# MCG-NJU/LinK

Measured on AMD Instinct MI355X. Metric: voxels/s through one LinK (3x7)^3 block, 100k active voxels C=64, higher is better.
Workload: dtype f32

## Files before the change

### link_amd/csrc/dense_batch_impl.h

```cpp
#include <stdlib.h>

#include <type_traits>
#include <vector>

#include "dense_batch_common.h"
#include "dense_gather.h"
#include "dense_io.h"

namespace DC_IO_NS {
using namespace link;

#include "dense_k1_impl.h"
#include "dense_k2_cfg.h"
#include "dense_gather_quad_impl.h"

static_assert(DC_ST_AUX == 16, "the S rows must leave the L2 (sc1) for the in-launch hand-off K1 -> K2");

struct dc_bt_frame_t {
  const void *feats; const int4 *coords; int4 *slots; uint32_t *cnt; int32_t *cell_n; int32_t *vcell; float *S; int32_t *hdr;
  void *out; int64_t n;
};
struct dc_bt_frames_t { dc_bt_frame_t f[DC_BT_MAX]; };
struct dc_bt_par_t {
  const float *w_pre, *pre_ln_w, *pre_ln_b, *w_pos, *ln_w, *ln_b;
// ... 143 lines not shown
struct dc_bt_k2_args_t {
  dc_bt_frames_t fr;
  dc_bt_par_t p;
  link_dc_grid_t g;
  int nframes, txn, tyn, zsplit, nwg, k1_target;
  int32_t *sync;
};

template <int OP, int R>
__global__ void __launch_bounds__(256 + 64 * (DC_K2Q_CW + (DC_K2Q_PMAP ? 1 : 0)), 4) k_dc_batch_k2(dc_bt_k2_args_t args_by_value) {
  (void)args_by_value;
#if defined(__HIP_DEVICE_COMPILE__)
  static_assert(DC_K2Q_PMAP == 1, "the mapper wave draws the items");
  typedef const __attribute__((address_space(4))) dc_bt_k2_args_t *args_ptr_t;
  constexpr unsigned CTL_THREAD = 256 + 64 * DC_K2Q_CW;
  __shared__ int s_ctl[2];
  const int x = (int)(__builtin_amdgcn_s_getreg((4 - 1) << 11 | 0 << 6 | 20) & 7u);
  int t_next = 0;
  if (threadIdx.x == CTL_THREAD) {
    args_ptr_t a = (args_ptr_t)__builtin_amdgcn_kernarg_segment_ptr();
    int32_t *sy = a->sync;
    const int per = (a->nwg + 7) >> 3;
    if (DC_BT_PROF)
      bt_row(a->p.dbg2, (unsigned long long)a->nframes * (8 * per) + blockIdx.x, 9999, 0, __builtin_amdgcn_s_memrealtime(), 0, 0, blockIdx.x);
    const int t = __hip_atomic_fetch_add(&sy[bt_cursor(x)], 1, __ATOMIC_RELAXED, __HIP_MEMORY_SCOPE_AGENT);
    t_next = __hip_atomic_fetch_add(&sy[bt_cursor(x)], 1, __ATOMIC_RELAXED, __HIP_MEMORY_SCOPE_AGENT);
    int f = t < a->nframes * per ? t / per : -1;
    if (f >= 0 && !bt_wait_ge(sy, bt_k1(f), a->k1_target)) f = -1;
    s_ctl[0] = f; s_ctl[1] = f >= 0 ? (t - f * per) * 8 + x : 0;
  }
  __syncthreads();
  for (;;) {
    args_ptr_t a = (args_ptr_t)__builtin_amdgcn_kernarg_segment_ptr();
    asm volatile("" : "+s"(a));
    const int f = __builtin_amdgcn_readfirstlane(s_ctl[0]), bid = __builtin_amdgcn_readfirstlane(s_ctl[1]);
    if (f < 0) break;
    const unsigned long long tq0 = DC_BT_PROF ? __builtin_amdgcn_s_memrealtime() : 0;
    __syncthreads();
    {
      const link_dc_grid_t g = a->g;
      unsigned tidx = threadIdx.x;
      asm volatile("" : "+v"(tidx));
      dc_k2q_body<OP, R, false, true>(a->fr.f[f].S, a->fr.f[f].cell_n, a->fr.f[f].slots, a->p.w_pos, nullptr, a->p.ln_w, a->p.ln_b, a->p.cg,
                                      1.0f, a->p.eps, a->fr.f[f].n, g, a->txn, a->tyn, a->zsplit, a->nwg, a->fr.f[f].out, nullptr, bid, tidx);
    }
    if (threadIdx.x == CTL_THREAD) {
      const unsigned long long tq1 = DC_BT_PROF ? __builtin_amdgcn_s_memrealtime() : 0;
      int32_t *sy = a->sync;
      const int per = (a->nwg + 7) >> 3;
      const int t = t_next;
      int fn = t < a->nframes * per ? t / per : -1;
      if (fn >= 0) {
        t_next = __hip_atomic_fetch_add(&sy[bt_cursor(x)], 1, __ATOMIC_RELAXED, __HIP_MEMORY_SCOPE_AGENT);
        if (!bt_wait_ge(sy, bt_k1(fn), a->k1_target)) fn = -1;
      }
      s_ctl[0] = fn; s_ctl[1] = fn >= 0 ? (t - fn * per) * 8 + x : 0;
      if (DC_BT_PROF) bt_row(a->p.dbg2, (unsigned long long)f * (8 * per) + bid, (unsigned long long)f, (unsigned long long)bid, tq0, tq1, __builtin_amdgcn_s_memrealtime(), (unsigned long long)blockIdx.x);
    }
    __syncthreads();
  }
#endif
}


template <int OP, int R>
static int batch_launch(const dc_bt_host_t &c, const dc_bt_frames_t &fr, const dc_bt_par_t &p, const link_dc_grid_t &g, const link_elk_desc_t &d,
                        int nframes, int64_t nmax) {
  using K1 = dc_k1_cfg<64, OP>;
  using KQ = dc_k2q_cfg<OP, R>;
  using KG = typename dc_k2_cfg<OP, R>::G;
  constexpr int LDS_GRAN = 1280, LDS_GRANS = 128, K1_STATIC = 256, K2_STATIC = 16;
  constexpr int k1_lds = 65 * LDS_GRAN - K1_STATIC;
  constexpr int k2_lds = KQ::LDS_BYTES;
  static_assert(k1_lds >= K1::LDS_BYTES && (k2_lds + K2_STATIC + LDS_GRAN - 1) / LDS_GRAN <= LDS_GRANS - 65, "LDS shaping of the two persistent roles");
  int32_t *sync = c.sync;
  const int64_t vi = (int64_t)g.dim[0] * g.dim[1] * g.dim[2] * g.dim[3];
  const int k1_wgs = c.cus;
  static const int rpw = [] { const char *e = getenv("LINK_DC_BATCH_RPW"); const int v = e ? atoi(e) : 1; return v < 1 ? 1 : (v > 16 ? 16 : v); }();
  int cpw = (int)((vi + (int64_t)k1_wgs * K1::NW * rpw - 1) / ((int64_t)k1_wgs * K1::NW * rpw));
  if (cpw < 1) cpw = 1;
  const int k1_target = (int)((vi + cpw - 1) / cpw);
  const int txn = (g.dim[0] + KG::TX - 1) / KG::TX, tyn = (g.dim[1] + KG::TY - 1) / KG::TY;
  static const int zs_env = [] { const char *e = getenv("LINK_DC_BATCH_ZSPLIT"); const int v = e ? atoi(e) : 1; return v < 1 ? 1 : (v > 8 ? 8 : v); }();
  int zsplit = zs_env;
  if (zsplit > g.dim[2]) zsplit = g.dim[2];
  const int64_t nwg = (int64_t)txn * tyn * g.dim[3] * zsplit;
  if (nwg > (1 << 20)) return LINK_ERR_ARG;
  int wpf = (int)((nmax + 255) / 256);
  if (wpf < 1) wpf = 1;
  (void)hipFuncSetAttribute(reinterpret_cast<const void *>(&k_dc_batch_k1<OP, 2>), hipFuncAttributeMaxDynamicSharedMemorySize, k1_lds);
  (void)hipFuncSetAttribute(reinterpret_cast<const void *>(&k_dc_batch_k2<OP, R>), hipFuncAttributeMaxDynamicSharedMemorySize, k2_lds);
  const int ins_wgs = c.cus;
  const dc_bt_ins_args_t a0{fr, g, nframes, wpf, sync};
  hipLaunchKernelGGL(k_dc_batch_insert, dim3((unsigned)ins_wgs * DC_BT_INS_WAVES), dim3(64), 0, c.sc, a0);
  int rc = check_launch("link_elk_core_dense_forward_batch (insert)");
  if (rc != LINK_OK) return rc;
  hipLaunchKernelGGL((k_dc_batch_k1<OP, 2>), dim3((unsigned)k1_wgs), dim3(64 * K1::NW), k1_lds, c.sa, fr, p, g, nframes, cpw, k1_target, wpf, sync);
  rc = check_launch("link_elk_core_dense_forward_batch (K1)");
  if (rc != LINK_OK) return rc;
  const dc_bt_k2_args_t a2{fr, p, g, nframes, txn, tyn, zsplit, (int)nwg, k1_target, sync};
  static_assert(sizeof(dc_bt_k2_args_t) <= 4096, "kernel arguments");
  hipLaunchKernelGGL((k_dc_batch_k2<OP, R>), dim3((unsigned)c.cus), dim3(KQ::THREADS), k2_lds, c.sb, a2);
  return check_launch("link_elk_core_dense_forward_batch (K2)");
}

int batch_set_launch(const dc_bt_host_t &c, const link_dc_buffers_t *frames, const int64_t *n, int nb, const link_dc_grid_t &g,
                     const link_elk_desc_t &d) {
  const link_dc_buffers_t &b0 = frames[0];
  const dc_bt_par_t p{b0.w_pre, b0.pre_ln_w, b0.pre_ln_b, b0.w_pos, b0.ln_w, b0.ln_b, d.cg, d.eps, c.dbg1, c.dbg2};
  dc_bt_frames_t fr{};
  int64_t nmax = 0;
  for (int i = 0; i < nb; i++) {
    const link_dc_buffers_t &b = frames[i];
    fr.f[i] = dc_bt_frame_t{b.feats, reinterpret_cast<const int4 *>(b.coords), reinterpret_cast<int4 *>(b.slots), b.cnt, b.cell_n, b.vcell, b.S,
                            b.hdr, b.out, n[i]};
    nmax = n[i] > nmax ? n[i] : nmax;
  }
  if (d.op == LINK_OP_COS) return d.r == 3 ? batch_launch<LINK_OP_COS, 3>(c, fr, p, g, d, nb, nmax) : batch_launch<LINK_OP_COS, 2>(c, fr, p, g, d, nb, nmax);
  return d.r == 3 ? batch_launch<LINK_OP_SIN, 3>(c, fr, p, g, d, nb, nmax) : batch_launch<LINK_OP_SIN, 2>(c, fr, p, g, d, nb, nmax);
}
}
```

### link_amd/csrc/dense_fused_impl.h

```cpp
#pragma once
#include <type_traits>

#include "dense_gather.h"
#include "dense_io.h"

namespace DC_IO_NS {
using namespace link;

#include "dense_k1_impl.h"

template <int C, int OP, int NB, bool PIPE>
static int launch_k1p(const link_dc_buffers_t *b, const link_dc_grid_t &g, const link_elk_desc_t &d, int64_t n,
                     bool warm, hipStream_t st) {
  using K = dc_k1_cfg<C, OP>;
  const int64_t vi = (int64_t)g.dim[0] * g.dim[1] * g.dim[2] * g.dim[3];
  int64_t waves = (int64_t)(b->tune.k1_wgs > 0 ? b->tune.k1_wgs : 512) * 4;
  int cpw = (int)((vi + waves - 1) / waves);
  if (cpw < 1) cpw = 1;
  const int64_t wgs = (vi + (int64_t)cpw * K::NW - 1) / ((int64_t)cpw * K::NW);
  int k1_pad = b->tune.k1_lds_pad;
  k1_pad = k1_pad < 0 ? 0 : (k1_pad > 16384 ? 16384 : k1_pad);
  const int lds_k1 = K::LDS_BYTES + k1_pad <= 160 * 1024 ? K::LDS_BYTES + k1_pad : K::LDS_BYTES;
  if (lds_k1 > 64 * 1024)
    (void)hipFuncSetAttribute(reinterpret_cast<const void *>(&k_dc_premix_modsum<C, OP, NB, PIPE>),
// ... 825 lines not shown
    (void)hipFuncSetAttribute(reinterpret_cast<const void *>(&k_dc_gather_demod_own<OP, R, PP, DD>),                  \
                              hipFuncAttributeMaxDynamicSharedMemorySize, KO::LDS_BYTES + k2_pad);                   \
    hipLaunchKernelGGL((k_dc_gather_demod_own<OP, R, PP, DD>), dim3((unsigned)grid), dim3(320), KO::LDS_BYTES + k2_pad, st, b->S, \
                       b->cell_n, reinterpret_cast<const int4 *>(b->slots), b->fin, b->w_pos, b->alpha, b->ln_w,      \
                       b->ln_b, d.cg, d.coord_div, d.eps, n, g, txn, tyn, zsplit, (int)nwg, b->out,                   \
                       reinterpret_cast<unsigned long long *>(b->tune.k2_dbg));                                       \
  } while (0)
    if (pair) { if (div) LINK_K2O(true, true); else LINK_K2O(true, false); }
    else { if (div) LINK_K2O(false, true); else LINK_K2O(false, false); }
#undef LINK_K2O
    return check_launch("link_dc_gather_demod");
  }
  if constexpr (dc_k2q_cfg<OP, R>::FITS) {
    if (pair && !b->alpha && !(b->tune.k2_form & 9) && !k2_single) {
      using KQ = dc_k2q_cfg<OP, R>;
#define LINK_K2Q(DD)                                                                                                  \
  do {                                                                                                                \
    (void)hipFuncSetAttribute(reinterpret_cast<const void *>(&k_dc_gather_demod_quad<OP, R, DD>),                     \
                              hipFuncAttributeMaxDynamicSharedMemorySize, KQ::LDS_BYTES + k2_pad);                   \
    hipLaunchKernelGGL((k_dc_gather_demod_quad<OP, R, DD>), dim3((unsigned)grid), dim3(KQ::THREADS), KQ::LDS_BYTES + k2_pad, st, b->S, \
                       b->cell_n, reinterpret_cast<const int4 *>(b->slots), b->w_pos, b->alpha, b->ln_w, b->ln_b, d.cg, \
                       d.coord_div, d.eps, n, g, txn, tyn, zsplit, (int)nwg, b->out,                                   \
                       reinterpret_cast<unsigned long long *>(b->tune.k2_dbg));                                       \
  } while (0)
      if (div) LINK_K2Q(true); else LINK_K2Q(false);
#undef LINK_K2Q
      return check_launch("link_dc_gather_demod");
    }
  }
  if (!(b->tune.k2_form & 1) && K2::SPLIT_FITS) {
    if (pair) { if (div) LINK_K2S(true, true); else LINK_K2S(true, false); }
    else { if (div) LINK_K2S(false, true); else LINK_K2S(false, false); }
    return check_launch("link_dc_gather_demod");
  }
#undef LINK_K2S
#define LINK_K2(PP, DD)                                                                                               \
  do {                                                                                                                \
// ... 55 lines not shown
```

### link_amd/csrc/dense_gather.h

```cpp
#pragma once
#include "dense_common.h"

namespace link {

template <int C, int P, int R>
struct dc_gather_cfg {
  static constexpr int LPR = C / 4;
  static constexpr int NG = 256 / LPR;
  static constexpr int TY = NG >= 64 ? 8 : (NG >= 16 ? 4 : 2);
  static constexpr int TX = NG / TY;
  static constexpr int HLO = (R == 3) ? 1 : 0;
  static constexpr int HX = TX + R - 1, HY = TY + R - 1;
  static constexpr int NCOL = HX * HY;
  static constexpr int RP = P * C / 4;
  static constexpr int NPC = NCOL * RP;
  static constexpr int PASSES = (NPC + 255) / 256;
  static constexpr int EPW = 64;
  static constexpr int NI = PASSES + 1;
  static constexpr int PLANE_BYTES = PASSES * 256 * 16;
  static constexpr int CNT_BYTES = 4 * 256;
  static constexpr int BUF_BYTES = PLANE_BYTES + CNT_BYTES;
  static constexpr int LDS_BYTES = 3 * BUF_BYTES;
  static_assert(NCOL <= 256, "count image: 4 waves x 64 entries");
  static_assert(NCOL * P * C * 4 + 3 * C * 4 < 65536, "ds_read immediate offsets are 16 bit");
};
// ... 57 lines not shown
        "ds_read_b32 %6, %9 offset:%c16\n\tds_read_b32 %7, %9 offset:%c17\n\t"
        "s_waitcnt lgkmcnt(0)"
        : "=&v"(v0), "=&v"(v1), "=&v"(v2), "=&v"(v3), "=&v"(v4), "=&v"(v5), "=&v"(n0), "=&v"(n1)
        : "v"(ra), "v"(ca), O_(0, 0), O_(0, 1), O_(0, 2), O_(1, 0), O_(1, 1), O_(1, 2), Q_(0), Q_(1)
        : "memory");
    const v4f_t a = v0 + v3, b = v1 + v4, d = v2 + v5;
    cur[0].x += a.x; cur[0].y += a.y; cur[0].z += a.z; cur[0].w += a.w;
    cur[1].x += b.x; cur[1].y += b.y; cur[1].z += b.z; cur[1].w += b.w;
    cur[P - 1].x += d.x; cur[P - 1].y += d.y; cur[P - 1].z += d.z; cur[P - 1].w += d.w;
  }
  cc += (float)n0 + (float)n1 + (float)n2;
#undef O_
#undef Q_
}

template <int C>
__device__ __forceinline__ void dc_read_plane_p2r3(uint32_t ra, uint32_t ca, float4 (&cur)[2], float &cc) {
  using K = dc_gather_cfg<C, 2, 3>;
  constexpr int RB = 2 * C * 4;
#define O_(dx, dy, pp) "i"((((dx) * K::HY + (dy)) * RB) + (pp) * C * 4)
#define Q_(dx, dy) "i"(((dx) * K::HY + (dy)) * 4)
  v4f_t a0, a1, a2, a3, a4, a5, b0, b1, b2, b3, b4, b5;
  int m0, m1, m2, n0, n1, n2;
  asm volatile(
      "ds_read_b128 %0, %18 offset:%c20\n\tds_read_b128 %1, %18 offset:%c21\n\t"
      "ds_read_b128 %2, %18 offset:%c22\n\tds_read_b128 %3, %18 offset:%c23\n\t"
      "ds_read_b128 %4, %18 offset:%c24\n\tds_read_b128 %5, %18 offset:%c25\n\t"
      "ds_read_b32 %6, %19 offset:%c26\n\tds_read_b32 %7, %19 offset:%c27\n\tds_read_b32 %8, %19 offset:%c28\n\t"
      "ds_read_b128 %9, %18 offset:%c29\n\tds_read_b128 %10, %18 offset:%c30\n\t"
      "ds_read_b128 %11, %18 offset:%c31\n\tds_read_b128 %12, %18 offset:%c32\n\t"
      "ds_read_b128 %13, %18 offset:%c33\n\tds_read_b128 %14, %18 offset:%c34\n\t"
      "ds_read_b32 %15, %19 offset:%c35\n\tds_read_b32 %16, %19 offset:%c36\n\tds_read_b32 %17, %19 offset:%c37\n\t"
      "s_waitcnt lgkmcnt(9)"
// ... 44 lines not shown
```

### link_amd/csrc/dense_gather_quad_impl.h

```cpp
#pragma once
#ifndef DC_K2_MAP
#define DC_K2_MAP 1
#endif

#ifndef DC_K2Q_CW
#define DC_K2Q_CW 3
#endif
#ifndef DC_K2Q_PMAP
#define DC_K2Q_PMAP 1
#endif
#ifndef DC_K2Q_EARLY
#define DC_K2Q_EARLY 1
#endif
#ifndef DC_K2Q_RIM
#define DC_K2Q_RIM 1
#endif
#ifndef DC_K2Q_FMA
#define DC_K2Q_FMA 1
#endif

template <int OP, int R>
struct dc_k2q_cfg {
  using K2 = dc_k2_cfg<OP, R>;
  static constexpr int PAR_OFF = K2::SPLIT_LDS_BYTES;
  static constexpr int MAP_OFF = PAR_OFF + 2 * 64 * 4;
  static constexpr int MAP_BYTES = 64 * 4 + 16;
  static constexpr int LDS_BYTES = MAP_OFF + (DC_K2Q_PMAP ? 3 * MAP_BYTES : 0);
  static constexpr int THREADS = 256 + 64 * (DC_K2Q_CW + (DC_K2Q_PMAP ? 1 : 0));
  static constexpr bool FITS = K2::P == 2 && 2 * LDS_BYTES <= 160 * 1024;
};

__device__ __forceinline__ void lds_rd9_b128(uint32_t ar, uint32_t a0, uint32_t a1, v4f_t &r, v4f_t (&x)[2][4]) {
  asm volatile("ds_read_b128 %0, %9\n\t"
               "ds_read_b128 %1, %10\n\tds_read_b128 %2, %10 offset:64\n\tds_read_b128 %3, %10 offset:128\n\tds_read_b128 %4, %10 offset:192\n\t"
               "ds_read_b128 %5, %11\n\tds_read_b128 %6, %11 offset:64\n\tds_read_b128 %7, %11 offset:128\n\tds_read_b128 %8, %11 offset:192\n\t"
               "s_waitcnt lgkmcnt(0)"
               : "=&v"(r), "=&v"(x[0][0]), "=&v"(x[0][1]), "=&v"(x[0][2]), "=&v"(x[0][3]), "=&v"(x[1][0]), "=&v"(x[1][1]),
                 "=&v"(x[1][2]), "=&v"(x[1][3])
// ... 48 lines not shown
    asm volatile("ds_read_b32 %0, %4\n\tds_read_b32 %1, %5\n\tds_read_b32 %2, %6\n\tds_read_b32 %3, %7\n\ts_waitcnt lgkmcnt(0)"
                 : "=&v"(cn[0]), "=&v"(cn[1]), "=&v"(cn[2]), "=&v"(cn[3])
                 : "v"(base + off[0]), "v"(base + off[1]), "v"(base + off[2]), "v"(base + off[3])
                 : "memory");
  } else {
#pragma unroll
    for (int i = 0; i < N; i++) cn[i] = lds_rd_b32(base + off[i]);
  }
}
__device__ __forceinline__ float dc_quad_sum(float v) {
  v += __builtin_bit_cast(float, __builtin_amdgcn_update_dpp(0, __builtin_bit_cast(int, v), 0xB1, 0xF, 0xF, true));
  v += __builtin_bit_cast(float, __builtin_amdgcn_update_dpp(0, __builtin_bit_cast(int, v), 0x4E, 0xF, 0xF, true));
  return v;
}

template <int OP, int R, bool DIV, bool COH = false>
__device__ __forceinline__ void dc_k2q_body(
    const float *__restrict__ S_, const int32_t *__restrict__ cell_n, const int4 *__restrict__ slots,
    const float *__restrict__ w_pos, const float *__restrict__ alpha, const float *__restrict__ ln_w,
    const float *__restrict__ ln_b, int cg, float coord_div, float eps, int64_t n, const link_dc_grid_t &g, int txn, int tyn,
    int zsplit, int nwg, void *__restrict__ out, unsigned long long *__restrict__ dbg, const int bid, const unsigned tidx) {
  using K2 = dc_k2_cfg<OP, R>;
  using KQ = dc_k2q_cfg<OP, R>;
  DC_PROF_PTR(dbg);
  unsigned long long tq0 = dbg ? DC_NOW() : 0, tq_dma = 0, tq_bar = 0, tq_work = 0;
  int tq_rounds = 0;
  using K = typename K2::G;
  constexpr int C = 64, P = 2, TY = K::TY, TX = K::TX, HY = K::HY, HLO = K::HLO;
  constexpr int RB = P * C * 4;
  static_assert(K2::P == 2, "two-part rows");
  extern __shared__ __attribute__((aligned(16))) char lds[];
  const bool producer = tidx < 256;
  const int tid = tidx & 255, lane = tid & 63, wave = __builtin_amdgcn_readfirstlane((tidx & 255) >> 6);
  const int per = (nwg + 7) >> 3;
  const int L = (bid & 7) * per + (bid >> 3);
  if (L >= nwg) return;
  int t = L;
  const int zseg = t % zsplit; t /= zsplit;
#if DC_K2_MAP
  const int per_b = txn * tyn;
  const int b = t / per_b;
  int tt2 = t - b * per_b;
  const int H = (tyn + 1) >> 1;
  int tx, ty;
  if (tt2 < txn * H) { tx = tt2 / H; ty = tt2 - tx * H; }
  else { tt2 -= txn * H; const int H2 = tyn - H; tx = tt2 / H2; ty = H + tt2 - tx * H2; }
#else
  const int ty = t % tyn; t /= tyn;
  const int tx = t % txn;
  const int b = t / txn;
#endif
  const int Dx = g.dim[0], Dy = g.dim[1], Dz = g.dim[2];
  const int PDx = g.pdim[0], PDy = g.pdim[1], PDz = g.pdim[2];
  const int x0 = tx * TX, y0 = ty * TY;
  const int zs = (int)(((long long)Dz * zseg) / zsplit), ze = (int)(((long long)Dz * (zseg + 1)) / zsplit);
  if (zs >= ze) return;
  const int nplanes = (ze - zs) + R - 1;
  const int pz0 = zs + 1 - HLO;
  const uint32_t lds_base = (uint32_t)(size_t)(__attribute__((address_space(3))) char *)lds;
  const uint32_t abuf0 = lds_base + K2::SPLIT_ABUF_OFF, ncnt0 = lds_base + K2::SPLIT_NCNT_OFF;
  if (tidx < 128) {
    float *par = reinterpret_cast<float *>(lds + KQ::PAR_OFF);
    par[tidx] = tidx < 64 ? ln_w[tidx] : ln_b[tidx - 64];
  }
  if (producer) {
    auto col_cell0 = [&](int hx, int hy) {
      int px = x0 + 1 - HLO + hx, py = y0 + 1 - HLO + hy;
      px = px < PDx - 1 ? px : PDx - 1;
      py = py < PDy - 1 ? py : PDy - 1;
// ... 18 lines not shown
    auto cnt_slot = [&](int plane, int pm3) -> uint32_t {
      (void)plane;
      return (uint32_t)(pm3 * K2::SPLIT_BUF_BYTES + K2::SPLIT_PLANE);
    };
    auto issue_cnt = [&](int plane, int pm3) {
      int pz = pz0 + plane;
      pz = pz < PDz - 1 ? pz : PDz - 1;
      const int32_t *csrc = cell_n + cnt_cell0 + pz;
      __builtin_amdgcn_global_load_lds((const __attribute__((address_space(1))) void *)csrc,
                                       (__attribute__((address_space(3))) void *)(lds + cnt_slot(plane, pm3) + wave * 256), 4, 0, COH ? 16 : 0);
    };
    uint32_t rec_cell0;
    int rec_k;
    {
      const int piece = wave * 16 + (lane & 15);
      const int col = piece >> 2;
      rec_k = piece & 3;
      rec_cell0 = col_cell0(col / TY + HLO, col % TY + HLO);
    }
    const char *Sb = reinterpret_cast<const char *>(S_);
    auto issue = [&](int plane, int pm3, bool) {
      int pz = pz0 + plane;
      pz = pz < PDz - 1 ? pz : PDz - 1;
      char *buf = lds + pm3 * K2::SPLIT_BUF_BYTES;
#pragma unroll
      for (int i = 0; i < K::PASSES; i++) {
        const bool surplus = (i * 256 + wave * 64) >= K::NPC;
        const int ii = surplus ? 0 : i;
        const char *src = Sb + (size_t)(surplus ? src_off[0] : src_off[i]) + (size_t)pz * RB;
        __builtin_amdgcn_global_load_lds((const __attribute__((address_space(1))) void *)src,
                                         (__attribute__((address_space(3))) void *)(buf + (ii * 256 + wave * 64) * 16), 16, 0, COH ? 16 : 0);
      }
      issue_cnt(plane, pm3);
      int po = pz0 + plane - (R - 1) + HLO;
      po = po < 0 ? 0 : (po < PDz - 1 ? po : PDz - 1);
      const int4 *rsrc = slots + ((size_t)(rec_cell0 + po) * DC_INL + rec_k);
      if (lane < 16)
        __builtin_amdgcn_global_load_lds((const __attribute__((address_space(1))) void *)rsrc,
                                         (__attribute__((address_space(3))) void *)(lds + K2::SPLIT_REC_OFF + (plane & 3) * K2::REC_BYTES + wave * 256), 16, 0, COH ? 16 : 0);
    };
    const int grp = tid >> 4, li = tid & 15;
    const bool rim_t = DC_K2Q_RIM && (y0 + TY > Dy) && (x0 + TX <= Dx);
    const int ix = rim_t ? grp % TX : grp / TY, iy = rim_t ? grp / TX : grp % TY;
    const int cell = ix * TY + iy;
    const bool col_ok = (x0 + ix < Dx) && (y0 + iy < Dy);
    const bool wave_has = (DC_K2Q_RIM && DC_K2Q_PMAP) ? __any(col_ok) : true;
    if (!wave_has && li == 0) {
      lds_wr_b32(ncnt0 + (uint32_t)(cell * 4), 0);
      lds_wr_b32(ncnt0 + (uint32_t)(K2::NG * 4 + cell * 4), 0);
    }
    const uint32_t row_lane = (uint32_t)((ix * HY + iy) * RB + li * 16);
    const uint32_t cnt_lane = (uint32_t)((ix * HY + iy) * 4);
    float4 r0[P], r1[P];
    float c0 = 0.f, c1 = 0.f;
    int n_prev = 0;
#pragma unroll
    for (int pp = 0; pp < P; pp++) r0[pp] = r1[pp] = make_float4(0.f, 0.f, 0.f, 0.f);
    issue(0, 0, false);
    if (nplanes > 1) issue(1, 1, false);
    int m3 = 0, m3p2 = 2;
// ... 5 lines not shown
      asm volatile("s_waitcnt lgkmcnt(0)" ::: "memory");
      if (dbg) { const unsigned long long tqb = DC_NOW(); tq_dma += tqb - tqa; tqa = tqb; }
      asm volatile("s_barrier" ::: "memory");
      if (dbg) { const unsigned long long tqb = DC_NOW(); tq_bar += tqb - tqa; tqa = tqb; }
      if (i >= nplanes) break;
      if (i + 2 < nplanes) issue(i + 2, m3p2, true);
      const uint32_t bufa = lds_base + (uint32_t)(m3 * K2::SPLIT_BUF_BYTES);
      if (!wave_has) continue;
      float4 cur[P];
      float cc = 0.f;
#pragma unroll
      for (int pp = 0; pp < P; pp++) cur[pp] = make_float4(0.f, 0.f, 0.f, 0.f);
      {
        const uint32_t ra = bufa + row_lane, ca = lds_base + cnt_slot(i, m3) + cnt_lane;
        if constexpr (R == 3) {
          dc_read_plane_p2r3<C>(ra, ca, cur, cc);
        } else {
          dc_read_dx<C, P, R, 0>(ra, ca, cur, cc);
          dc_read_dx<C, P, R, 1>(ra, ca, cur, cc);
        }
      }
      const int n_here = lds_rd_b32(lds_base + cnt_slot(i, m3) + cnt_lane + (uint32_t)((HLO * HY + HLO) * 4));
      if (i >= R - 1) {
        const uint32_t abuf = abuf0 + (uint32_t)((i & 1) * K2::NG * RB), ncnt = ncnt0 + (uint32_t)((i & 1) * K2::NG * 4);
        float4 a[P];
        float den;
        if (R == 3) {
          den = (c0 + c1) + cc;
#pragma unroll
          for (int pp = 0; pp < P; pp++) {
            a[pp].x = (r0[pp].x + r1[pp].x) + cur[pp].x; a[pp].y = (r0[pp].y + r1[pp].y) + cur[pp].y;
// ... 22 lines not shown
    }
    if (dbg && lane == 0) {
      unsigned long long *d = dbg + ((size_t)L * 8 + (tidx >> 6)) * 8;
      d[0] = DC_NOW() - tq0; d[1] = tq_dma; d[2] = tq_bar; d[3] = tq_work; d[4] = tq0; d[5] = 0; d[6] = nplanes; d[7] = 1;
    }
    return;
  }
  constexpr int CW = DC_K2Q_CW, SLOTS = 16 * CW;
  if (DC_K2Q_PMAP && wave == CW) {
    int m3 = 0;
    for (int i = 0; i <= nplanes; i++, m3 = m3 == 2 ? 0 : m3 + 1) {
      asm volatile("s_barrier" ::: "memory");
      if (i >= nplanes) break;
      const uint32_t ca = lds_base + (uint32_t)(m3 * K2::SPLIT_BUF_BYTES + K2::SPLIT_PLANE);
      int run = 0, c_ = 0, start = 0;
#define Q_(k) "i"(((((k) / TY) + HLO) * HY + ((k) % TY) + HLO) * 4)
#define DC_MAP4(K0)                                                                                                          \
      {                                                                                                                      \
        int n0, n1, n2, n3;                                                                                                  \
        asm volatile("ds_read_b32 %0, %4 offset:%c5\n\tds_read_b32 %1, %4 offset:%c6\n\tds_read_b32 %2, %4 offset:%c7\n\t"     \
                     "ds_read_b32 %3, %4 offset:%c8\n\ts_waitcnt lgkmcnt(0)"                                                \
                     : "=&v"(n0), "=&v"(n1), "=&v"(n2), "=&v"(n3)                                                            \
                     : "v"(ca), Q_(K0), Q_(K0 + 1), Q_(K0 + 2), Q_(K0 + 3)                                                   \
                     : "memory");                                                                                            \
        const int nn[4] = {n0, n1, n2, n3};                                                                                  \
        _Pragma("unroll") for (int kk = 0; kk < 4; kk++) {                                                                   \
          const int k = K0 + kk;                                                                                             \
          const bool okk = (x0 + k / TY < Dx) && (y0 + k % TY < Dy);    \
          run += okk ? nn[kk] : 0;                                                                                           \
          if (k < 15) {                                                                                                      \
            const bool le = run <= lane;                                                                                     \
            c_ += le ? 1 : 0;                                                                                                \
            start = le ? run : start;                                                                                        \
          }                                                                                                                  \
        }                                                                                                                    \
      }
      DC_MAP4(0) DC_MAP4(4) DC_MAP4(8) DC_MAP4(12)
#undef DC_MAP4
#undef Q_
      const uint32_t mb = lds_base + (uint32_t)(KQ::MAP_OFF + m3 * KQ::MAP_BYTES);
      lds_wr_b32(mb + (uint32_t)(lane * 4), (c_ << 12) | ((lane - start) & 4095));
      if (lane == 0) lds_wr_b32(mb + 256u, run);
      asm volatile("s_waitcnt lgkmcnt(0)" ::: "memory");
    }
    return;
  }
  const int q = lane & 3, li16 = lane & 15;
  const int qd = wave * 16 + (lane >> 2);
  const __amdgpu_buffer_rsrc_t r_out = dc_rsrc(out, (uint32_t)(n * C * IO_BYTES));
  float w0[2][4], w1[2][4], w2[2][4];
#pragma unroll
  for (int j = 0; j < 2; j++)
#pragma unroll
    for (int e = 0; e < 4; e++) {
// ... 152 lines not shown
      for (int j = 0; j < 4; j++) {
        float4 o;
        o.x = (nv[j][0] - mean) * rs * gwb[0][j][0] + gwb[1][j][0]; o.y = (nv[j][1] - mean) * rs * gwb[0][j][1] + gwb[1][j][1];
        o.z = (nv[j][2] - mean) * rs * gwb[0][j][2] + gwb[1][j][2]; o.w = (nv[j][3] - mean) * rs * gwb[0][j][3] + gwb[1][j][3];
        io_st4(r_out, (uint32_t)rec.w * (uint32_t)C + (uint32_t)(16 * j + 4 * q), valid, o);
      }
    }
    if (dbg) tq_work += DC_NOW() - tqa;
  }
  if (dbg && lane == 0) {
    unsigned long long *d = dbg + ((size_t)L * 8 + (tidx >> 6)) * 8;
    d[0] = DC_NOW() - tq0; d[1] = tq0; d[2] = tq_bar; d[3] = 0; d[4] = tq_work; d[5] = tq_rounds; d[6] = nplanes; d[7] = 2;
  }
}

template <int OP, int R, bool DIV>
__global__ void __launch_bounds__(256 + 64 * (DC_K2Q_CW + (DC_K2Q_PMAP ? 1 : 0)), 4) k_dc_gather_demod_quad(
    const float *__restrict__ S_, const int32_t *__restrict__ cell_n, const int4 *__restrict__ slots,
    const float *__restrict__ w_pos, const float *__restrict__ alpha, const float *__restrict__ ln_w,
    const float *__restrict__ ln_b, int cg, float coord_div, float eps, int64_t n, link_dc_grid_t g, int txn, int tyn,
    int zsplit, int nwg, void *__restrict__ out, unsigned long long *__restrict__ dbg) {
  dc_k2q_body<OP, R, DIV>(S_, cell_n, slots, w_pos, alpha, ln_w, ln_b, cg, coord_div, eps, n, g, txn, tyn, zsplit, nwg, out, dbg,
                          (int)blockIdx.x, threadIdx.x);
}
```

### link_amd/csrc/dense_k2_cfg.h

```cpp
#pragma once

template <int OP, int R>
struct dc_k2_cfg {
  static constexpr int C = 64, LPR = 16, NG = 16;
  static constexpr int P = (OP == LINK_OP_COSX) ? 3 : 2;
  using G = dc_gather_cfg<C, P, R>;
  static constexpr int RB = P * C * 4;
  static constexpr int REC_OFF = G::PLANE_BYTES + G::CNT_BYTES;
  static constexpr int REC_BYTES = NG * DC_INL * 16;
  static constexpr int BUF_BYTES = REC_OFF + REC_BYTES;
  static constexpr int ABUF_OFF = 3 * BUF_BYTES;
  static constexpr int NCNT_OFF = ABUF_OFF + NG * RB;
  static constexpr int LDS_BYTES = NCNT_OFF + NG * 4;
  static constexpr int SPLIT_PLANE = G::NPC * 16;
  static constexpr int SPLIT_BUF_BYTES = SPLIT_PLANE + G::CNT_BYTES;
  static constexpr int SPLIT_ABUF_OFF = 3 * SPLIT_BUF_BYTES;
  static constexpr int SPLIT_NCNT_OFF = SPLIT_ABUF_OFF + 2 * NG * RB;
  static constexpr int SPLIT_REC_OFF = SPLIT_NCNT_OFF + 2 * NG * 4;
  static constexpr int SPLIT_LDS_BYTES = SPLIT_REC_OFF + 4 * REC_BYTES;
  static constexpr bool SPLIT_FITS = 2 * SPLIT_LDS_BYTES <= 160 * 1024;
  static constexpr int NI = G::PASSES + 2;
  static_assert(G::NG == NG && G::TX * G::TY == NG, "16 columns");
};

__device__ __forceinline__ void lds_rd2_b128(uint32_t a0, uint32_t a1, v4f_t &x0, v4f_t &x1) {
  asm volatile("ds_read_b128 %0, %2\n\tds_read_b128 %1, %3\n\ts_waitcnt lgkmcnt(0)" : "=&v"(x0), "=&v"(x1) : "v"(a0), "v"(a1) : "memory");
}
__device__ __forceinline__ void lds_rd6_b128(uint32_t a0, uint32_t a1, uint32_t a2, uint32_t a3, uint32_t a4, uint32_t a5,
                                             v4f_t &x0, v4f_t &x1, v4f_t &x2, v4f_t &x3, v4f_t &x4, v4f_t &x5) {
  asm volatile("ds_read_b128 %0, %6\n\tds_read_b128 %1, %7\n\tds_read_b128 %2, %8\n\tds_read_b128 %3, %9\n\t"
               "ds_read_b128 %4, %10\n\tds_read_b128 %5, %11\n\ts_waitcnt lgkmcnt(0)"
               : "=&v"(x0), "=&v"(x1), "=&v"(x2), "=&v"(x3), "=&v"(x4), "=&v"(x5)
               : "v"(a0), "v"(a1), "v"(a2), "v"(a3), "v"(a4), "v"(a5)
               : "memory");
}
__device__ __forceinline__ int lds_rd_b32(uint32_t a) {
  int v;
// ... 11 lines not shown
```

### link_amd/elk.py

```python
from __future__ import annotations

import ctypes
import weakref
import math
from typing import Dict, Optional, Tuple

import torch
import torch.nn as nn
import torch.nn.functional as TF

from . import _lib as L
from .aggregate import _AuxToVoxel, _BlockMean, link_index_of
from .functional import sphash, sphashquery
from .index import BlockIndex, GridTooLarge, box_neighbor_map, foreign_neighbor_map, strided_out_coords, transpose_table
from .tensor import SparseTensor
from .utils import get_kernel_offsets, make_ntuple

__all__ = ["ELKBlock", "TSELKBlock", "Conv3d", "spconv2ts", "ts2spconv", "SparseConvTensor",
           "elk_core_fused", "elk_core_autograd", "elk_core_train", "ElkCorePlan", "subm_conv", "subm_conv_ln_add_relu",
           "invalidate_derived_weights", "release_block_driver"]

_OPS = {"cos": L.OP_COS, "sin": L.OP_SIN, "cos_x": L.OP_COSX}
_IO_DTYPES = {torch.float32: L.IO_F32, torch.float16: L.IO_F16, torch.bfloat16: L.IO_BF16}

# ... 237 lines not shown
                                                int(self._n_prev) if build_index else 0, int(bool(build_index)), st)
        if build_index and rc == 0:
            self._cur, self._n_prev = cur, n
        return rc

    def set_tuning(self, **kw):
        if not self.dense:
            if kw:
                raise L.LinkAmdError("ElkCorePlan.set_tuning: only the dense-cell layout has per-plan launch geometry "
                                     "(general layout: ElkCorePlan(..., tiles=False) selects the four-kernel form)")
            return self
        t = self.buf.tune
        multi = self.frames_in_flight > 1
        t.k1_wgs, t.k2_zsplit = (256, 2) if multi else (512, 0)
        t.k1_lds_pad = t.k2_lds_pad = t.k1_form = t.k2_form = t.mode = 0
        if not multi and not self.sparse and self.c in (32, 64) and self.baseop != "cos_x" and "k1_form" not in kw:
            t.k1_form = 2
            if "k1_wgs" not in kw:
                t.k1_wgs = 1024
        for k, v in kw.items():
            if k not in ("k1_wgs", "k2_zsplit", "k1_lds_pad", "k2_lds_pad", "k1_form", "k2_form", "mode", "k1_dbg", "k2_dbg"):
                raise L.LinkAmdError(f"ElkCorePlan.set_tuning: unknown key {k!r}")
            setattr(t, k, v)
        if t.k1_form == 0 and multi and "k1_lds_pad" not in kw:
            t.k1_lds_pad = 2048
        return self

    def _init_general(self):
        device, n_cap, c = self.device, self.n_cap, self.c
        v = self.grid.cells
# ... 118 lines not shown


class ElkCoreBatch:

    def __init__(self, frames: int, n_cap: int, c: int, baseop: str, cg: int, r: int, s: int, bounds, device, eps: float = 1e-6,
                 slot_cap: int = 0, share: Optional["ElkCoreBatch"] = None):
        if c != 64 or cg != 32 or baseop not in ("cos", "sin") or r not in (2, 3):
            raise L.LinkAmdError("ElkCoreBatch: C = 64, cg = 32, cos / sin, r in {2, 3} (include/link_amd.h section H)")
        if frames < 1:
            raise ValueError("ElkCoreBatch: at least one frame")
        self.plans = [ElkCorePlan(n_cap, c, baseop, cg, r, s, bounds, device, eps=eps, layout="dense", slot_cap=slot_cap)
                      for _ in range(frames)]
        if int(self.plans[0].dcg.k) > 352:
            raise L.LinkAmdError("ElkCoreBatch: slot capacity above 352")
        self.n_cap, self.c, self.device = n_cap, c, device
        self._bufs = (L.LinkDcBuffers * frames)()
        self._n = (ctypes.c_int64 * frames)()
        if share is not None:
            self._ctx, self._owner = share._ctx, share
        else:
            h = ctypes.c_void_p()
            with torch.cuda.device(device):
                L.check(L.lib().link_dc_batch_create(ctypes.byref(h)), "link_dc_batch_create")
            self._ctx, self._owner = h, None
        self._fn = L.lib().link_elk_core_dense_forward_batch

    def __del__(self):
        try:
            if getattr(self, "_owner", None) is None and getattr(self, "_ctx", None):
                L.lib().link_dc_batch_destroy(self._ctx)
# ... 1747 lines not shown
```

Measured before the change: 3.114 billion.

## Cover ragged grid rims with 1x10 / 10x1 strip tiles in the quad gather

When a grid dimension is 4k+1 (r=3), the K2 quad gather now tiles the bulk with 4x4 tiles and covers the last row or column with thin 1x10 or 10x1 strip tiles. This avoids a whole row of mostly empty 4x4 tiles. Strips reuse the square tile's LDS layout, and lanes past the strip length are clamped or masked. The batch kernel's control state moves into LDS. Strips are on by default in the batch path but turned off for single plans (k2_form=16), and the single-plan path now also derives zsplit from the tile count.

New measurement: 3.275 billion, median of 6. 5.2% higher.

```diff
diff --git a/link_amd/csrc/dense_batch_impl.h b/link_amd/csrc/dense_batch_impl.h
--- a/link_amd/csrc/dense_batch_impl.h
+++ b/link_amd/csrc/dense_batch_impl.h
@@ -181,9 +181,8 @@
   static_assert(DC_K2Q_PMAP == 1, "the mapper wave draws the items");
   typedef const __attribute__((address_space(4))) dc_bt_k2_args_t *args_ptr_t;
   constexpr unsigned CTL_THREAD = 256 + 64 * DC_K2Q_CW;
-  __shared__ int s_ctl[2];
+  __shared__ int s_ctl[4];
   const int x = (int)(__builtin_amdgcn_s_getreg((4 - 1) << 11 | 0 << 6 | 20) & 7u);
-  int t_next = 0;
   if (threadIdx.x == CTL_THREAD) {
     args_ptr_t a = (args_ptr_t)__builtin_amdgcn_kernarg_segment_ptr();
     int32_t *sy = a->sync;
@@ -191,7 +190,8 @@
     if (DC_BT_PROF)
       bt_row(a->p.dbg2, (unsigned long long)a->nframes * (8 * per) + blockIdx.x, 9999, 0, __builtin_amdgcn_s_memrealtime(), 0, 0, blockIdx.x);
     const int t = __hip_atomic_fetch_add(&sy[bt_cursor(x)], 1, __ATOMIC_RELAXED, __HIP_MEMORY_SCOPE_AGENT);
-    t_next = __hip_atomic_fetch_add(&sy[bt_cursor(x)], 1, __ATOMIC_RELAXED, __HIP_MEMORY_SCOPE_AGENT);
+    s_ctl[2] = __hip_atomic_fetch_add(&sy[bt_cursor(x)], 1, __ATOMIC_RELAXED, __HIP_MEMORY_SCOPE_AGENT);
+    s_ctl[3] = x;
     int f = t < a->nframes * per ? t / per : -1;
     if (f >= 0 && !bt_wait_ge(sy, bt_k1(f), a->k1_target)) f = -1;
     s_ctl[0] = f; s_ctl[1] = f >= 0 ? (t - f * per) * 8 + x : 0;
@@ -215,13 +215,13 @@
       const unsigned long long tq1 = DC_BT_PROF ? __builtin_amdgcn_s_memrealtime() : 0;
       int32_t *sy = a->sync;
       const int per = (a->nwg + 7) >> 3;
-      const int t = t_next;
+      const int t = s_ctl[2], xc = s_ctl[3];
       int fn = t < a->nframes * per ? t / per : -1;
       if (fn >= 0) {
-        t_next = __hip_atomic_fetch_add(&sy[bt_cursor(x)], 1, __ATOMIC_RELAXED, __HIP_MEMORY_SCOPE_AGENT);
+        s_ctl[2] = __hip_atomic_fetch_add(&sy[bt_cursor(xc)], 1, __ATOMIC_RELAXED, __HIP_MEMORY_SCOPE_AGENT);
         if (!bt_wait_ge(sy, bt_k1(fn), a->k1_target)) fn = -1;
       }
-      s_ctl[0] = fn; s_ctl[1] = fn >= 0 ? (t - fn * per) * 8 + x : 0;
+      s_ctl[0] = fn; s_ctl[1] = fn >= 0 ? (t - fn * per) * 8 + xc : 0;
       if (DC_BT_PROF) bt_row(a->p.dbg2, (unsigned long long)f * (8 * per) + bid, (unsigned long long)f, (unsigned long long)bid, tq0, tq1, __builtin_amdgcn_s_memrealtime(), (unsigned long long)blockIdx.x);
     }
     __syncthreads();
@@ -232,10 +232,9 @@
 
 template <int OP, int R>
 static int batch_launch(const dc_bt_host_t &c, const dc_bt_frames_t &fr, const dc_bt_par_t &p, const link_dc_grid_t &g, const link_elk_desc_t &d,
-                        int nframes, int64_t nmax) {
+                        int nframes, int64_t nmax, bool strips) {
   using K1 = dc_k1_cfg<64, OP>;
   using KQ = dc_k2q_cfg<OP, R>;
-  using KG = typename dc_k2_cfg<OP, R>::G;
   constexpr int LDS_GRAN = 1280, LDS_GRANS = 128, K1_STATIC = 256, K2_STATIC = 16;
   constexpr int k1_lds = 65 * LDS_GRAN - K1_STATIC;
   constexpr int k2_lds = KQ::LDS_BYTES;
@@ -247,11 +246,11 @@
   int cpw = (int)((vi + (int64_t)k1_wgs * K1::NW * rpw - 1) / ((int64_t)k1_wgs * K1::NW * rpw));
   if (cpw < 1) cpw = 1;
   const int k1_target = (int)((vi + cpw - 1) / cpw);
-  const int txn = (g.dim[0] + KG::TX - 1) / KG::TX, tyn = (g.dim[1] + KG::TY - 1) / KG::TY;
+  const dc_k2q_tiles_t tq = dc_k2q_tiles(g, R, strips);
   static const int zs_env = [] { const char *e = getenv("LINK_DC_BATCH_ZSPLIT"); const int v = e ? atoi(e) : 1; return v < 1 ? 1 : (v > 8 ? 8 : v); }();
   int zsplit = zs_env;
   if (zsplit > g.dim[2]) zsplit = g.dim[2];
-  const int64_t nwg = (int64_t)txn * tyn * g.dim[3] * zsplit;
+  const int64_t nwg = ((int64_t)tq.txn * tq.tyn + tq.nxs + tq.nys) * g.dim[3] * zsplit;
   if (nwg > (1 << 20)) return LINK_ERR_ARG;
   int wpf = (int)((nmax + 255) / 256);
   if (wpf < 1) wpf = 1;
@@ -265,7 +264,7 @@
   hipLaunchKernelGGL((k_dc_batch_k1<OP, 2>), dim3((unsigned)k1_wgs), dim3(64 * K1::NW), k1_lds, c.sa, fr, p, g, nframes, cpw, k1_target, wpf, sync);
   rc = check_launch("link_elk_core_dense_forward_batch (K1)");
   if (rc != LINK_OK) return rc;
-  const dc_bt_k2_args_t a2{fr, p, g, nframes, txn, tyn, zsplit, (int)nwg, k1_target, sync};
+  const dc_bt_k2_args_t a2{fr, p, g, nframes, tq.txn, tq.tyn, zsplit, (int)nwg, k1_target, sync};
   static_assert(sizeof(dc_bt_k2_args_t) <= 4096, "kernel arguments");
   hipLaunchKernelGGL((k_dc_batch_k2<OP, R>), dim3((unsigned)c.cus), dim3(KQ::THREADS), k2_lds, c.sb, a2);
   return check_launch("link_elk_core_dense_forward_batch (K2)");
@@ -283,7 +282,9 @@
                             b.hdr, b.out, n[i]};
     nmax = n[i] > nmax ? n[i] : nmax;
   }
-  if (d.op == LINK_OP_COS) return d.r == 3 ? batch_launch<LINK_OP_COS, 3>(c, fr, p, g, d, nb, nmax) : batch_launch<LINK_OP_COS, 2>(c, fr, p, g, d, nb, nmax);
-  return d.r == 3 ? batch_launch<LINK_OP_SIN, 3>(c, fr, p, g, d, nb, nmax) : batch_launch<LINK_OP_SIN, 2>(c, fr, p, g, d, nb, nmax);
-}
-}
+  static const bool sq_env = [] { const char *e = getenv("LINK_DC_BATCH_SQUARE_RIM"); return e && atoi(e) != 0; }();
+  const bool strips = !(b0.tune.k2_form & 16) && !sq_env;
+  if (d.op == LINK_OP_COS) return d.r == 3 ? batch_launch<LINK_OP_COS, 3>(c, fr, p, g, d, nb, nmax, strips) : batch_launch<LINK_OP_COS, 2>(c, fr, p, g, d, nb, nmax, strips);
+  return d.r == 3 ? batch_launch<LINK_OP_SIN, 3>(c, fr, p, g, d, nb, nmax, strips) : batch_launch<LINK_OP_SIN, 2>(c, fr, p, g, d, nb, nmax, strips);
+}
+}
diff --git a/link_amd/csrc/dense_fused_impl.h b/link_amd/csrc/dense_fused_impl.h
--- a/link_amd/csrc/dense_fused_impl.h
+++ b/link_amd/csrc/dense_fused_impl.h
@@ -863,13 +863,22 @@
   if constexpr (dc_k2q_cfg<OP, R>::FITS) {
     if (pair && !b->alpha && !(b->tune.k2_form & 9) && !k2_single) {
       using KQ = dc_k2q_cfg<OP, R>;
+      const dc_k2q_tiles_t tq = dc_k2q_tiles(g, R, !(b->tune.k2_form & 16));
+      const int64_t tiles = ((int64_t)tq.txn * tq.tyn + tq.nxs + tq.nys) * g.dim[3];
+      int zq = b->tune.k2_zsplit;
+      if (zq <= 0) {
+        zq = (int)(512 / tiles);
+        if (zq < 1) zq = 1;
+      }
+      if (zq > g.dim[2]) zq = g.dim[2];
+      const int64_t nwg_q = tiles * zq, grid_q = (nwg_q + 7) / 8 * 8;
 #define LINK_K2Q(DD)                                                                                                  \
   do {                                                                                                                \
     (void)hipFuncSetAttribute(reinterpret_cast<const void *>(&k_dc_gather_demod_quad<OP, R, DD>),                     \
                               hipFuncAttributeMaxDynamicSharedMemorySize, KQ::LDS_BYTES + k2_pad);                   \
-    hipLaunchKernelGGL((k_dc_gather_demod_quad<OP, R, DD>), dim3((unsigned)grid), dim3(KQ::THREADS), KQ::LDS_BYTES + k2_pad, st, b->S, \
+    hipLaunchKernelGGL((k_dc_gather_demod_quad<OP, R, DD>), dim3((unsigned)grid_q), dim3(KQ::THREADS), KQ::LDS_BYTES + k2_pad, st, b->S, \
                        b->cell_n, reinterpret_cast<const int4 *>(b->slots), b->w_pos, b->alpha, b->ln_w, b->ln_b, d.cg, \
-                       d.coord_div, d.eps, n, g, txn, tyn, zsplit, (int)nwg, b->out,                                   \
+                       d.coord_div, d.eps, n, g, tq.txn, tq.tyn, zq, (int)nwg_q, b->out,                               \
                        reinterpret_cast<unsigned long long *>(b->tune.k2_dbg));                                       \
   } while (0)
       if (div) LINK_K2Q(true); else LINK_K2Q(false);
diff --git a/link_amd/csrc/dense_gather.h b/link_amd/csrc/dense_gather.h
--- a/link_amd/csrc/dense_gather.h
+++ b/link_amd/csrc/dense_gather.h
@@ -3,12 +3,13 @@
 
 namespace link {
 
-template <int C, int P, int R>
+template <int C, int P, int R, int TX_ = 0, int TY_ = 0>
 struct dc_gather_cfg {
   static constexpr int LPR = C / 4;
   static constexpr int NG = 256 / LPR;
-  static constexpr int TY = NG >= 64 ? 8 : (NG >= 16 ? 4 : 2);
-  static constexpr int TX = NG / TY;
+  static constexpr int TY = TY_ > 0 ? TY_ : (NG >= 64 ? 8 : (NG >= 16 ? 4 : 2));
+  static constexpr int TX = TX_ > 0 ? TX_ : NG / TY;
+  static_assert(TX * TY <= NG, "an output column per lane group");
   static constexpr int HLO = (R == 3) ? 1 : 0;
   static constexpr int HX = TX + R - 1, HY = TY + R - 1;
   static constexpr int NCOL = HX * HY;
@@ -96,9 +97,9 @@
 #undef Q_
 }
 
-template <int C>
+template <int C, int TX_ = 0, int TY_ = 0>
 __device__ __forceinline__ void dc_read_plane_p2r3(uint32_t ra, uint32_t ca, float4 (&cur)[2], float &cc) {
-  using K = dc_gather_cfg<C, 2, 3>;
+  using K = dc_gather_cfg<C, 2, 3, TX_, TY_>;
   constexpr int RB = 2 * C * 4;
 #define O_(dx, dy, pp) "i"((((dx) * K::HY + (dy)) * RB) + (pp) * C * 4)
 #define Q_(dx, dy) "i"(((dx) * K::HY + (dy)) * 4)
diff --git a/link_amd/csrc/dense_gather_quad_impl.h b/link_amd/csrc/dense_gather_quad_impl.h
--- a/link_amd/csrc/dense_gather_quad_impl.h
+++ b/link_amd/csrc/dense_gather_quad_impl.h
@@ -19,9 +19,9 @@
 #define DC_K2Q_FMA 1
 #endif
 
-template <int OP, int R>
+template <int OP, int R, int TX_ = 0, int TY_ = 0>
 struct dc_k2q_cfg {
-  using K2 = dc_k2_cfg<OP, R>;
+  using K2 = dc_k2_cfg<OP, R, TX_, TY_>;
   static constexpr int PAR_OFF = K2::SPLIT_LDS_BYTES;
   static constexpr int MAP_OFF = PAR_OFF + 2 * 64 * 4;
   static constexpr int MAP_BYTES = 64 * 4 + 16;
@@ -100,45 +100,35 @@
   return v;
 }
 
-template <int OP, int R, bool DIV, bool COH = false>
-__device__ __forceinline__ void dc_k2q_body(
+template <int SH> struct dc_k2q_shape { static constexpr int TX = 0, TY = 0; };
+template <> struct dc_k2q_shape<1> { static constexpr int TX = 1, TY = 10; };
+template <> struct dc_k2q_shape<2> { static constexpr int TX = 10, TY = 1; };
+#define DC_K2Q_STRIP 10
+
+template <int OP, int R, bool DIV, bool COH, int SH>
+__device__ __forceinline__ void dc_k2q_tile(
     const float *__restrict__ S_, const int32_t *__restrict__ cell_n, const int4 *__restrict__ slots,
     const float *__restrict__ w_pos, const float *__restrict__ alpha, const float *__restrict__ ln_w,
-    const float *__restrict__ ln_b, int cg, float coord_div, float eps, int64_t n, const link_dc_grid_t &g, int txn, int tyn,
-    int zsplit, int nwg, void *__restrict__ out, unsigned long long *__restrict__ dbg, const int bid, const unsigned tidx) {
-  using K2 = dc_k2_cfg<OP, R>;
-  using KQ = dc_k2q_cfg<OP, R>;
+    const float *__restrict__ ln_b, int cg, float coord_div, float eps, int64_t n, const link_dc_grid_t &g, const int b, const int x0,
+    const int y0, const int zseg, int zsplit, void *__restrict__ out,
+    unsigned long long *__restrict__ dbg, const int L, const unsigned tidx) {
+  using K2 = dc_k2_cfg<OP, R, dc_k2q_shape<SH>::TX, dc_k2q_shape<SH>::TY>;
+  using KQ = dc_k2q_cfg<OP, R, dc_k2q_shape<SH>::TX, dc_k2q_shape<SH>::TY>;
+  static_assert(K2::G::HX * K2::G::HY <= 36 && K2::G::TX * K2::G::TY <= K2::NG, "a tile shape within the 4 x 4 tile's halo and lane groups");
+  static_assert(KQ::LDS_BYTES == dc_k2q_cfg<OP, R>::LDS_BYTES && K2::NI == dc_k2_cfg<OP, R>::NI, "every shape runs in the square tile's LDS layout");
   DC_PROF_PTR(dbg);
   unsigned long long tq0 = dbg ? DC_NOW() : 0, tq_dma = 0, tq_bar = 0, tq_work = 0;
   int tq_rounds = 0;
   using K = typename K2::G;
   constexpr int C = 64, P = 2, TY = K::TY, TX = K::TX, HY = K::HY, HLO = K::HLO;
+  constexpr int NT = TX * TY;
   constexpr int RB = P * C * 4;
   static_assert(K2::P == 2, "two-part rows");
   extern __shared__ __attribute__((aligned(16))) char lds[];
   const bool producer = tidx < 256;
   const int tid = tidx & 255, lane = tid & 63, wave = __builtin_amdgcn_readfirstlane((tidx & 255) >> 6);
-  const int per = (nwg + 7) >> 3;
-  const int L = (bid & 7) * per + (bid >> 3);
-  if (L >= nwg) return;
-  int t = L;
-  const int zseg = t % zsplit; t /= zsplit;
-#if DC_K2_MAP
-  const int per_b = txn * tyn;
-  const int b = t / per_b;
-  int tt2 = t - b * per_b;
-  const int H = (tyn + 1) >> 1;
-  int tx, ty;
-  if (tt2 < txn * H) { tx = tt2 / H; ty = tt2 - tx * H; }
-  else { tt2 -= txn * H; const int H2 = tyn - H; tx = tt2 / H2; ty = H + tt2 - tx * H2; }
-#else
-  const int ty = t % tyn; t /= tyn;
-  const int tx = t % txn;
-  const int b = t / txn;
-#endif
-  const int Dx = g.dim[0], Dy = g.dim[1], Dz = g.dim[2];
+  const int Dx = g.dim[0] - ((SH == 2 && (g.dim[0] & 3) == 1) ? 1 : 0), Dy = g.dim[1], Dz = g.dim[2];
   const int PDx = g.pdim[0], PDy = g.pdim[1], PDz = g.pdim[2];
-  const int x0 = tx * TX, y0 = ty * TY;
   const int zs = (int)(((long long)Dz * zseg) / zsplit), ze = (int)(((long long)Dz * (zseg + 1)) / zsplit);
   if (zs >= ze) return;
   const int nplanes = (ze - zs) + R - 1;
@@ -187,7 +177,8 @@
     int rec_k;
     {
       const int piece = wave * 16 + (lane & 15);
-      const int col = piece >> 2;
+      int col = piece >> 2;
+      if constexpr (NT < K2::NG) col = col < NT ? col : NT - 1;
       rec_k = piece & 3;
       rec_cell0 = col_cell0(col / TY + HLO, col % TY + HLO);
     }
@@ -213,10 +204,15 @@
                                          (__attribute__((address_space(3))) void *)(lds + K2::SPLIT_REC_OFF + (plane & 3) * K2::REC_BYTES + wave * 256), 16, 0, COH ? 16 : 0);
     };
     const int grp = tid >> 4, li = tid & 15;
-    const bool rim_t = DC_K2Q_RIM && (y0 + TY > Dy) && (x0 + TX <= Dx);
-    const int ix = rim_t ? grp % TX : grp / TY, iy = rim_t ? grp / TX : grp % TY;
-    const int cell = ix * TY + iy;
-    const bool col_ok = (x0 + ix < Dx) && (y0 + iy < Dy);
+    const bool rim_t = DC_K2Q_RIM && SH == 0 && (y0 + TY > Dy) && (x0 + TX <= Dx);
+    int ix = rim_t ? grp % TX : grp / TY, iy = rim_t ? grp / TX : grp % TY;
+    bool grp_ok = true;
+    if constexpr (NT < K2::NG) {
+      grp_ok = grp < NT;
+      ix = grp_ok ? ix : 0; iy = grp_ok ? iy : 0;
+    }
+    const int cell = grp_ok ? ix * TY + iy : grp;
+    const bool col_ok = grp_ok && (x0 + ix < Dx) && (y0 + iy < Dy);
     const bool wave_has = (DC_K2Q_RIM && DC_K2Q_PMAP) ? __any(col_ok) : true;
     if (!wave_has && li == 0) {
       lds_wr_b32(ncnt0 + (uint32_t)(cell * 4), 0);
@@ -252,7 +248,7 @@
       {
         const uint32_t ra = bufa + row_lane, ca = lds_base + cnt_slot(i, m3) + cnt_lane;
         if constexpr (R == 3) {
-          dc_read_plane_p2r3<C>(ra, ca, cur, cc);
+          dc_read_plane_p2r3<C, dc_k2q_shape<SH>::TX, dc_k2q_shape<SH>::TY>(ra, ca, cur, cc);
         } else {
           dc_read_dx<C, P, R, 0>(ra, ca, cur, cc);
           dc_read_dx<C, P, R, 1>(ra, ca, cur, cc);
@@ -305,7 +301,8 @@
       if (i >= nplanes) break;
       const uint32_t ca = lds_base + (uint32_t)(m3 * K2::SPLIT_BUF_BYTES + K2::SPLIT_PLANE);
       int run = 0, c_ = 0, start = 0;
-#define Q_(k) "i"(((((k) / TY) + HLO) * HY + ((k) % TY) + HLO) * 4)
+#define QK_(k) ((k) < NT ? (k) : 0)
+#define Q_(k) "i"((((QK_(k) / TY) + HLO) * HY + (QK_(k) % TY) + HLO) * 4)
 #define DC_MAP4(K0)                                                                                                          \
       {                                                                                                                      \
         int n0, n1, n2, n3;                                                                                                  \
@@ -317,7 +314,7 @@
         const int nn[4] = {n0, n1, n2, n3};                                                                                  \
         _Pragma("unroll") for (int kk = 0; kk < 4; kk++) {                                                                   \
           const int k = K0 + kk;                                                                                             \
-          const bool okk = (x0 + k / TY < Dx) && (y0 + k % TY < Dy);    \
+          const bool okk = k < NT && (x0 + k / TY < Dx) && (y0 + k % TY < Dy);    \
           run += okk ? nn[kk] : 0;                                                                                           \
           if (k < 15) {                                                                                                      \
             const bool le = run <= lane;                                                                                     \
@@ -329,6 +326,7 @@
       DC_MAP4(0) DC_MAP4(4) DC_MAP4(8) DC_MAP4(12)
 #undef DC_MAP4
 #undef Q_
+#undef QK_
       const uint32_t mb = lds_base + (uint32_t)(KQ::MAP_OFF + m3 * KQ::MAP_BYTES);
       lds_wr_b32(mb + (uint32_t)(lane * 4), (c_ << 12) | ((lane - start) & 4095));
       if (lane == 0) lds_wr_b32(mb + 256u, run);
@@ -511,6 +509,61 @@
   }
 }
 
+struct dc_k2q_tiles_t { int txn, tyn, nxs, nys; };
+static inline dc_k2q_tiles_t dc_k2q_tiles(const link_dc_grid_t &g, int r, bool strips) {
+  const bool sx = strips && r == 3 && (g.dim[0] & 3) == 1, sy = strips && r == 3 && (g.dim[1] & 3) == 1;
+  const int dxs = g.dim[0] - (sx ? 1 : 0), dys = g.dim[1] - (sy ? 1 : 0);
+  return dc_k2q_tiles_t{(dxs + 3) / 4, (dys + 3) / 4, sx ? (g.dim[1] + DC_K2Q_STRIP - 1) / DC_K2Q_STRIP : 0,
+                        sy ? (dxs + DC_K2Q_STRIP - 1) / DC_K2Q_STRIP : 0};
+}
+
+template <int OP, int R, bool DIV, bool COH = false>
+__device__ __forceinline__ void dc_k2q_body(
+    const float *__restrict__ S_, const int32_t *__restrict__ cell_n, const int4 *__restrict__ slots,
+    const float *__restrict__ w_pos, const float *__restrict__ alpha, const float *__restrict__ ln_w,
+    const float *__restrict__ ln_b, int cg, float coord_div, float eps, int64_t n, const link_dc_grid_t &g, int txn, int tyn,
+    int zsplit, int nwg, void *__restrict__ out, unsigned long long *__restrict__ dbg, const int bid, const unsigned tidx) {
+  using KS = typename dc_k2_cfg<OP, R>::G;
+  const int per = (nwg + 7) >> 3;
+  const int L = (bid & 7) * per + (bid >> 3);
+  if (L >= nwg) return;
+  int t = L;
+  const int zseg = t % zsplit; t /= zsplit;
+  const bool sx = txn * KS::TX < g.dim[0], sy = tyn * KS::TY < g.dim[1];
+  const int per_b = txn * tyn;
+  const int nsq = per_b * g.dim[3];
+  if (R != 3 || t < nsq) {
+#if DC_K2_MAP
+    const int b = t / per_b;
+    int tt2 = t - b * per_b;
+    const int H = (tyn + 1) >> 1;
+    int tx, ty;
+    if (tt2 < txn * H) { tx = tt2 / H; ty = tt2 - tx * H; }
+    else { tt2 -= txn * H; const int H2 = tyn - H; tx = tt2 / H2; ty = H + tt2 - tx * H2; }
+#else
+    const int ty = t % tyn; t /= tyn;
+    const int tx = t % txn;
+    const int b = t / txn;
+#endif
+    dc_k2q_tile<OP, R, DIV, COH, 0>(S_, cell_n, slots, w_pos, alpha, ln_w, ln_b, cg, coord_div, eps, n, g, b, tx * KS::TX, ty * KS::TY, zseg, zsplit,
+                                    out, dbg, L, tidx);
+    return;
+  }
+  if constexpr (R == 3) {
+    const int dxs = g.dim[0] - (sx ? 1 : 0);
+    const int nxs = sx ? (g.dim[1] + DC_K2Q_STRIP - 1) / DC_K2Q_STRIP : 0, nys = sy ? (dxs + DC_K2Q_STRIP - 1) / DC_K2Q_STRIP : 0;
+    int u = t - nsq;
+    const int b = u / (nxs + nys);
+    u -= b * (nxs + nys);
+    if (u < nxs)
+      dc_k2q_tile<OP, R, DIV, COH, 1>(S_, cell_n, slots, w_pos, alpha, ln_w, ln_b, cg, coord_div, eps, n, g, b, g.dim[0] - 1, u * DC_K2Q_STRIP,
+                                      zseg, zsplit, out, dbg, L, tidx);
+    else
+      dc_k2q_tile<OP, R, DIV, COH, 2>(S_, cell_n, slots, w_pos, alpha, ln_w, ln_b, cg, coord_div, eps, n, g, b, (u - nxs) * DC_K2Q_STRIP,
+                                      g.dim[1] - 1, zseg, zsplit, out, dbg, L, tidx);
+  }
+}
+
 template <int OP, int R, bool DIV>
 __global__ void __launch_bounds__(256 + 64 * (DC_K2Q_CW + (DC_K2Q_PMAP ? 1 : 0)), 4) k_dc_gather_demod_quad(
     const float *__restrict__ S_, const int32_t *__restrict__ cell_n, const int4 *__restrict__ slots,
diff --git a/link_amd/csrc/dense_k2_cfg.h b/link_amd/csrc/dense_k2_cfg.h
--- a/link_amd/csrc/dense_k2_cfg.h
+++ b/link_amd/csrc/dense_k2_cfg.h
@@ -1,10 +1,10 @@
 #pragma once
 
-template <int OP, int R>
+template <int OP, int R, int TX_ = 0, int TY_ = 0>
 struct dc_k2_cfg {
   static constexpr int C = 64, LPR = 16, NG = 16;
   static constexpr int P = (OP == LINK_OP_COSX) ? 3 : 2;
-  using G = dc_gather_cfg<C, P, R>;
+  using G = dc_gather_cfg<C, P, R, TX_, TY_>;
   static constexpr int RB = P * C * 4;
   static constexpr int REC_OFF = G::PLANE_BYTES + G::CNT_BYTES;
   static constexpr int REC_BYTES = NG * DC_INL * 16;
@@ -20,7 +20,7 @@
   static constexpr int SPLIT_LDS_BYTES = SPLIT_REC_OFF + 4 * REC_BYTES;
   static constexpr bool SPLIT_FITS = 2 * SPLIT_LDS_BYTES <= 160 * 1024;
   static constexpr int NI = G::PASSES + 2;
-  static_assert(G::NG == NG && G::TX * G::TY == NG, "16 columns");
+  static_assert(G::NG == NG && G::TX * G::TY <= NG && (TX_ > 0 || G::TX * G::TY == NG), "16 columns");
 };
 
 __device__ __forceinline__ void lds_rd2_b128(uint32_t a0, uint32_t a1, v4f_t &x0, v4f_t &x1) {
diff --git a/link_amd/elk.py b/link_amd/elk.py
--- a/link_amd/elk.py
+++ b/link_amd/elk.py
@@ -275,6 +275,7 @@
         multi = self.frames_in_flight > 1
         t.k1_wgs, t.k2_zsplit = (256, 2) if multi else (512, 0)
         t.k1_lds_pad = t.k2_lds_pad = t.k1_form = t.k2_form = t.mode = 0
+        t.k2_form = 16
         if not multi and not self.sparse and self.c in (32, 64) and self.baseop != "cos_x" and "k1_form" not in kw:
             t.k1_form = 2
             if "k1_wgs" not in kw:
@@ -423,6 +424,8 @@
         if int(self.plans[0].dcg.k) > 352:
             raise L.LinkAmdError("ElkCoreBatch: slot capacity above 352")
         self.n_cap, self.c, self.device = n_cap, c, device
+        for p in self.plans:
+            p.buf.tune.k2_form = 0
         self._bufs = (L.LinkDcBuffers * frames)()
         self._n = (ctypes.c_int64 * frames)()
         if share is not None:
```
